# linnanwang/FastGen

Measured on AMD Instinct MI355X. Metric: images/sec at 4-step distilled (DMD2) sampling, higher is better.
Workload: dtype fp32 (tensors, accumulate) with split-bf16 x3 MFMA conv products

## Files before the change

fastgen_amd/csrc/conv.h:

```cpp
#pragma once
#include <hip/hip_runtime.h>

struct ConvArgs {
    const void* src1;
    const void* src2;
    int C1, C2;
    int Hs, Ws;
    int H, W;
    int B;
    const float2* ab;
    const void* wpack;
    const void* wpack_ws;
    const float* bias;
    const float* temb;
    int temb_stride;
    const void* resid;
    float scale;
    void* out;
    int Cout;
    float2* stats;
    int dbg;
    void* q_out;
    void* k_out;
    void* vt_out;
    const float* gate = nullptr;
    int gate_stride = 0;
    int act = 0;
    int heads = 0, head_dim = 0;
    size_t heads_lo_off = 0;
};

enum { PRO_NONE = 0, PRO_GN = 1, PRO_GN_SILU = 2 };
enum { RES_NONE = 0, RES_DOWN = 1, RES_UP = 2 };
enum { OUT_NHWC = 0, OUT_QKV = 1, OUT_TOK = 2, OUT_HEADS = 3 };

int launch_conv_fused(int dtype, int ks, int pro, int res, int outmode, const ConvArgs& a, hipStream_t stream);
int conv_stat_slots(int W);
bool conv_ws_supported(int dtype, int ks, int pro, int res, int outmode, const ConvArgs& a);
bool conv_ws_enabled();
int launch_conv_ws(int res, const ConvArgs& a, hipStream_t stream, bool prepare_only, int pro = PRO_GN_SILU);
bool conv_ws_shape_ok(int dtype, int cout, int cin, int res);
int launch_pack_conv_weights_ws(const float* w_oihw, void* wpack_ws, int cout, int cin, hipStream_t stream);
bool conv_x3ws_supported(int ks, int pro, int res, int outmode, const ConvArgs& a);
bool conv_x3ws_shape_ok(int cout, int cin, int res);
int conv_x3ws_stat_slots(int W);
int launch_conv_x3ws(int res, const ConvArgs& a, hipStream_t stream, bool prepare_only, int pro = PRO_GN_SILU);
int launch_pack_conv_weights_x3ws(const float* w_oihw, void* wpack_ws, int cout, int cin, hipStream_t stream);
int conv_launch_stat_slots(int dtype, int ks, int pro, int res, int outmode, const ConvArgs& a);
int launch_conv_ws_debug(const ConvArgs& a, int abl, hipStream_t stream);
int launch_conv_debug(int dtype, const ConvArgs& a, hipStream_t stream);
int conv_prepare_all(int dtype);
size_t conv_pack_elems(int cout, int cin, int ks);
int launch_pack_conv_weights(int dtype, const float* w_oihw, void* wpack, int cout, int cin, int ks, int qkv_perm,
                             hipStream_t stream);
```

fastgen_amd/csrc/conv_ws3.hip:

```cpp
#include "common.h"
#include "conv.h"

namespace {

constexpr int X3_NTHR = 768;
constexpr int X3_KC = 32;
constexpr int X3_PA = 16;
constexpr int X3_PLANE = 3072;
constexpr int X3_ABUF = 8 * X3_PLANE;
constexpr int X3_RING = 4;
constexpr int X3_HOFF = 128 * 512;
constexpr int X3_LDS = X3_HOFF + X3_RING * X3_ABUF;
constexpr int X3_STEPB = 9 * 2048;

template <int LOGW>
struct X3Geom {
    static constexpr int W = 1 << LOGW;
    static constexpr int TW = 16, TH = 8;
    static constexpr int TCOLS = W / TW;
    static constexpr int TPI = (W / TH) * TCOLS;
    static constexpr int HW_ = TW + 2, HH_ = TH + 2;
    static constexpr int HALO_PIX = HW_ * HH_;
    static constexpr int RS = HW_ * X3_PA;
};

__device__ __forceinline__ void x3_barrier() {
    asm volatile("s_waitcnt lgkmcnt(0)\n\ts_barrier" ::: "memory");
}

struct X3Frag {
    bf16x8 hi, lo;
};

template <int RES, int LOGW, int PRO>
__global__ __launch_bounds__(X3_NTHR) void conv3_x3ws_kernel(const ConvArgs a, const int ntiles) {
    using G = X3Geom<LOGW>;
    extern __shared__ __attribute__((aligned(16))) char smem[];
    char* const hbuf = smem;
    char* const ring = smem + X3_HOFF;

    const int tid = threadIdx.x;
    const int lane = tid & 63;
    const int wave = __builtin_amdgcn_readfirstlane(tid >> 6);
    const int Cin = a.C1 + a.C2;
    const int nchunk = Cin / X3_KC;
    const int G8 = (int)gridDim.x >> 3;
    const int wg = ((gridDim.x & 7) == 0) ? ((int)blockIdx.x & 7) * G8 + ((int)blockIdx.x >> 3) : (int)blockIdx.x;
    const int gstride = (int)gridDim.x;
    const int my_tiles = (ntiles - wg + gstride - 1) / gstride;
    const int S = my_tiles * nchunk;
    const int NSTEP = S + 3;
    const int H = a.H;

    if (wave < 8) {
        const int grp = wave >> 2, wl = wave & 3;
        const int col = lane & 15, g4 = lane >> 4;
        const size_t wstride = (size_t)nchunk * 9 * 1024;
        const __amdgpu_buffer_rsrc_t wrs = __builtin_amdgcn_make_buffer_rsrc(
            const_cast<__bf16*>(reinterpret_cast<const __bf16*>(a.wpack_ws) + (size_t)(grp * 8 + wl * 2) * wstride), 0, 0x7fffffff,
            0x00020000);
        const int wvoff = lane * 16;
        const int wsb = (int)(wstride * 2);
        auto load_w = [&](int byte_off) -> X3Frag {
            X3Frag f;
            f.hi = __builtin_bit_cast(bf16x8, __builtin_amdgcn_raw_buffer_load_b128(wrs, wvoff, byte_off, 0));
            f.lo = __builtin_bit_cast(bf16x8, __builtin_amdgcn_raw_buffer_load_b128(wrs, wvoff, byte_off + 1024, 0));
            return f;
        };
        X3Frag wq[3][2];
#pragma unroll
        for (int j = 0; j < 3; ++j)
#pragma unroll
            for (int nt = 0; nt < 2; ++nt) wq[j][nt] = load_w(nt * wsb + j * 2048);

        f32x4 acc[8][2];
#pragma unroll
        for (int m = 0; m < 8; ++m)
#pragma unroll
            for (int nt = 0; nt < 2; ++nt) acc[m][nt] = f32x4{0.f, 0.f, 0.f, 0.f};

        const int lane_off = g4 * X3_PLANE + col * X3_PA;
        const int dl0 = col * 512 + ((8 * wl + ((g4) ^ (col & 7))) << 4);
        const int dl1 = col * 512 + ((8 * wl + ((4 + g4) ^ (col & 7))) << 4);

        x3_barrier();
        int c = 0;
        for (int s = 0; s < NSTEP; ++s) {
            const int ls = s - 2 * grp;
            if (ls >= 0 && ls < S) {
                const char* abase = ring + (ls & 3) * X3_ABUF + lane_off;
                const int cn = (c + 1 == nchunk) ? 0 : c + 1;
                const int wcur = c * X3_STEPB;
                const int wnxt = (ls + 1 < S) ? cn * X3_STEPB : wcur;
                auto read_x = [&](int q, X3Frag (&xf)[2]) {
                    const int tap = q >> 2, m0 = 2 * (q & 3);
                    const int off = (tap / 3 + m0) * G::RS + (tap % 3) * X3_PA;
#pragma unroll
                    for (int m = 0; m < 2; ++m) {
                        xf[m].hi = *reinterpret_cast<const bf16x8*>(abase + off + m * G::RS);
                        xf[m].lo = *reinterpret_cast<const bf16x8*>(abase + off + m * G::RS + 4 * X3_PLANE);
                    }
                };
                auto mma12 = [&](int q, const X3Frag (&xf)[2]) {
                    const int tap = q >> 2, m0 = 2 * (q & 3);
                    const X3Frag(&wf)[2] = wq[tap % 3];
#pragma unroll
                    for (int m = 0; m < 2; ++m)
#pragma unroll
                        for (int nt = 0; nt < 2; ++nt)
                            acc[m0 + m][nt] = __builtin_amdgcn_mfma_f32_16x16x32_bf16(wf[nt].hi, xf[m].lo, acc[m0 + m][nt], 0, 0, 0);
#pragma unroll
                    for (int m = 0; m < 2; ++m)
#pragma unroll
                        for (int nt = 0; nt < 2; ++nt)
                            acc[m0 + m][nt] = __builtin_amdgcn_mfma_f32_16x16x32_bf16(wf[nt].lo, xf[m].hi, acc[m0 + m][nt], 0, 0, 0);
#pragma unroll
                    for (int m = 0; m < 2; ++m)
#pragma unroll
                        for (int nt = 0; nt < 2; ++nt)
                            acc[m0 + m][nt] = __builtin_amdgcn_mfma_f32_16x16x32_bf16(wf[nt].hi, xf[m].hi, acc[m0 + m][nt], 0, 0, 0);
                    if ((q & 3) != 3) return;
                    const int pn = (tap + 3 < 9) ? wcur + (tap + 3) * 2048 : wnxt + (tap + 3 - 9) * 2048;
#pragma unroll
                    for (int nt = 0; nt < 2; ++nt) wq[tap % 3][nt] = load_w(pn + nt * wsb);
                };
                X3Frag x0[2], x1[2];
                read_x(0, x0);
#pragma unroll
                for (int q = 0; q < 36; q += 2) {
                    read_x(q + 1, x1);
                    __builtin_amdgcn_sched_barrier(0);
                    mma12(q, x0);
                    __builtin_amdgcn_sched_barrier(0);
                    if (q + 2 < 36) read_x(q + 2, x0);
                    __builtin_amdgcn_sched_barrier(0);
                    mma12(q + 1, x1);
                    __builtin_amdgcn_sched_barrier(0);
                }
                if (c + 1 == nchunk) {
#pragma unroll
                    for (int m = 0; m < 8; ++m) {
                        *reinterpret_cast<f32x4*>(hbuf + m * 8192 + dl0) = acc[m][0];
                        *reinterpret_cast<f32x4*>(hbuf + m * 8192 + dl1) = acc[m][1];
                        acc[m][0] = f32x4{0.f, 0.f, 0.f, 0.f};
                        acc[m][1] = f32x4{0.f, 0.f, 0.f, 0.f};
                    }
                }
                c = cn;
            }
            x3_barrier();
        }
        return;
    }

    const int ptid = tid - 512;
    const int pw = wave - 8;
    const int oct = ptid & 3;
    const float* src1 = reinterpret_cast<const float*>(a.src1);
    const float* src2 = reinterpret_cast<const float*>(a.src2);
    int hdy[3], hdx[3], hlds[3];
#pragma unroll
    for (int i = 0; i < 3; ++i) {
        const int hq = min((ptid >> 2) + 64 * i, G::HALO_PIX - 1);
        const int hy = hq / G::HW_, hx = hq - hy * G::HW_;
        hdy[i] = hy - 1;
        hdx[i] = hx - 1;
        hlds[i] = oct * X3_PLANE + hy * G::RS + hx * X3_PA;
    }
    const bool third = (ptid >> 2) + 128 < G::HALO_PIX;

    auto tile_coord = [&](int t, int& n, int& slot, int& row0, int& col0) {
        n = t / G::TPI;
        slot = t - n * G::TPI;
        row0 = (slot / G::TCOLS) * G::TH;
        col0 = (slot % G::TCOLS) * G::TW;
    };

    struct Staged {
        f32x4 raw[3][2];
        float2 ab[8];
    };
    unsigned off1[3], off2[3];
    bool valid[3];
    const float2* abn = a.ab;
    auto tile_setup = [&](int t) __attribute__((always_inline)) {
        int n, slot, row0, col0;
        tile_coord(t, n, slot, row0, col0);
#pragma unroll
        for (int i = 0; i < 3; ++i) {
            const int y = row0 + hdy[i], x = col0 + hdx[i];
            valid[i] = (y >= 0) && (y < H) && (x >= 0) && (x < G::W) && (i < 2 || third);
            const int yc = min(max(y, 0), H - 1), xc = min(max(x, 0), G::W - 1);
            const int sy = (RES == RES_UP) ? (yc >> 1) : yc, sx = (RES == RES_UP) ? (xc >> 1) : xc;
            const unsigned pix = (unsigned)((n * a.Hs + sy) * a.Ws + sx);
            off1[i] = (pix * (unsigned)a.C1 + oct * 8) * 4u;
            off2[i] = (pix * (unsigned)a.C2 + oct * 8) * 4u;
        }
        abn = a.ab + (size_t)n * Cin;
    };
    auto stage_load = [&](Staged& st, int t, int c32) __attribute__((always_inline)) {
        if (c32 == 0) tile_setup(t);
        const bool first = c32 * X3_KC < a.C1;
        const char* base = first ? reinterpret_cast<const char*>(src1) + c32 * (X3_KC * 4)
                                 : reinterpret_cast<const char*>(src2) + (c32 * X3_KC - a.C1) * 4;
#pragma unroll
        for (int i = 0; i < 3; ++i) {
            const char* p = base + (first ? off1[i] : off2[i]);
            st.raw[i][0] = *reinterpret_cast<const f32x4*>(p);
            st.raw[i][1] = *reinterpret_cast<const f32x4*>(p + 16);
        }
        if (PRO == PRO_NONE) return;
        const float2* p = abn + c32 * X3_KC + oct * 8;
#pragma unroll
        for (int j = 0; j < 8; j += 2) {
            const f32x4 q = *reinterpret_cast<const f32x4*>(p + j);
            st.ab[j] = make_float2(q[0], q[1]);
            st.ab[j + 1] = make_float2(q[2], q[3]);
        }
    };
    auto stage_store = [&](const Staged& st, char* abuf) __attribute__((always_inline)) {
#pragma unroll
        for (int i = 0; i < 3; ++i) {
            float v[8];
#pragma unroll
            for (int j = 0; j < 8; ++j) {
                v[j] = st.raw[i][j >> 2][j & 3];
                if (PRO != PRO_NONE) v[j] = silu_f<true>(fmaf(v[j], st.ab[j].x, st.ab[j].y));
            }
            bf16x8 hi, lo;
            split8(v, hi, lo);
            typedef __attribute__((ext_vector_type(4))) unsigned u32x4;
            u32x4 wh = __builtin_bit_cast(u32x4, hi), wl_ = __builtin_bit_cast(u32x4, lo);
#pragma unroll
            for (int j = 0; j < 4; ++j) {
                wh[j] = valid[i] ? wh[j] : 0u;
                wl_[j] = valid[i] ? wl_[j] : 0u;
            }
            if (i < 2 || third) {
                *reinterpret_cast<u32x4*>(abuf + hlds[i]) = wh;
                *reinterpret_cast<u32x4*>(abuf + hlds[i] + 4 * X3_PLANE) = wl_;
            }
        }
    };

    const int chq = lane & 31, psub = lane >> 5;
    float* const out = reinterpret_cast<float*>(a.out);
    const float* const resid = reinterpret_cast<const float*>(a.resid);
    const bool has_resid = __builtin_amdgcn_readfirstlane(resid != nullptr);
    auto retire_half = [&](int t, int half) __attribute__((always_inline)) {
        int n, slot, row0, col0;
        tile_coord(t, n, slot, row0, col0);
        const int co = half * 128 + chq * 4;
        f32x4 radd = {0.f, 0.f, 0.f, 0.f};
        if (a.bias) radd = *reinterpret_cast<const f32x4*>(a.bias + co);
        if (a.temb) radd += *reinterpret_cast<const f32x4*>(a.temb + (size_t)n * a.temb_stride + co);
        radd *= a.scale;
        const size_t tb = (((size_t)n * H + row0) * G::W + col0) * 256 + co;
        float ssum = 0.f, ssq = 0.f;
#pragma unroll 1
        for (int grp8 = 0; grp8 < 2; ++grp8) {
            f32x4 rr[8], dv[8];
            unsigned go[8];
#pragma unroll
            for (int j = 0; j < 8; ++j) {
                const int px = pw * 32 + 2 * (grp8 * 8 + j) + psub;
                go[j] = (unsigned)(((px >> 4) * G::W + (px & 15)) * 256);
                rr[j] = f32x4{0.f, 0.f, 0.f, 0.f};
                if (has_resid) rr[j] = *reinterpret_cast<const f32x4*>(resid + tb + go[j]);
                dv[j] = *reinterpret_cast<const f32x4*>(hbuf + px * 512 + ((chq ^ (px & 7)) << 4));
            }
#pragma unroll
            for (int j = 0; j < 8; ++j) {
                f32x4 v;
#pragma unroll
                for (int e = 0; e < 4; ++e) v[e] = fmaf(dv[j][e], a.scale, radd[e]);
                if (has_resid) {
#pragma unroll
                    for (int e = 0; e < 4; ++e) v[e] = fmaf(rr[j][e], a.scale, v[e]);
                }
                *reinterpret_cast<f32x4*>(out + tb + go[j]) = v;
                ssum += (v[0] + v[1]) + (v[2] + v[3]);
                ssq += (v[0] * v[0] + v[1] * v[1]) + (v[2] * v[2] + v[3] * v[3]);
            }
        }
        ssum += __shfl_xor(ssum, 32);
        ssq += __shfl_xor(ssq, 32);
        if (a.stats && psub == 0) a.stats[(((size_t)n * G::TPI + slot) * 4 + pw) * 64 + half * 32 + chq] = make_float2(ssum, ssq);
    };

    auto advance = [&](int& t, int& cc) {
        if (++cc == nchunk) {
            cc = 0;
            t += gstride;
        }
    };
    Staged st;
    int t1 = wg, c1 = 0;
    stage_load(st, t1, c1);
    stage_store(st, ring);
    advance(t1, c1);
    x3_barrier();
    int sa = 0;
    for (int s = 0; s < NSTEP; ++s) {
        const bool more = s + 1 < S;
        if (more) stage_load(st, t1, c1);
        if (sa == 0 && s >= nchunk && s <= S) retire_half(wg + (s / nchunk - 1) * gstride, 0);
        if (sa == 2 % nchunk && s - 2 >= nchunk && s - 2 <= S && (s - 2) % nchunk == 0) retire_half(wg + ((s - 2) / nchunk - 1) * gstride, 1);
        if (more) {
            stage_store(st, ring + ((s + 1) & 3) * X3_ABUF);
            advance(t1, c1);
        }
        if (++sa == nchunk) sa = 0;
        x3_barrier();
    }
}

__global__ void pack_conv_weights_x3ws_kernel(const float* __restrict__ w, __bf16* __restrict__ out, int cout, int cin) {
    const size_t total = (size_t)cout * cin * 9;
    const int nstep = cin / X3_KC;
    for (size_t idx = (size_t)blockIdx.x * blockDim.x + threadIdx.x; idx < total; idx += (size_t)gridDim.x * blockDim.x) {
        size_t t = idx;
        const int j = t % 8; t /= 8;
        const int lane = t % 64; t /= 64;
        const int tap = t % 9; t /= 9;
        const int step = t % nstep; t /= nstep;
        const int n16 = (int)t;
        const int co = n16 * 16 + (lane & 15);
        const int ci = step * X3_KC + 8 * (lane >> 4) + j;
        const float v = w[((size_t)co * cin + ci) * 9 + tap];
        const __bf16 hi = (__bf16)v;
        const size_t o = (idx / 512) * 1024 + (idx % 512);
        out[o] = hi;
        out[o + 512] = (__bf16)(v - (float)hi);
    }
}

int g_x3_cus[16] = {};

template <int RES, int LOGW, int PRO>
int launch_x3_one(const ConvArgs& a, hipStream_t stream, bool prepare_only) {
    using G = X3Geom<LOGW>;
    auto kern = conv3_x3ws_kernel<RES, LOGW, PRO>;
    int dev = 0;
    if (hipGetDevice(&dev) != hipSuccess || dev < 0 || dev >= 16) return (int)hipErrorInvalidDevice;
    static bool attr_done[16] = {};
    if (!attr_done[dev]) {
        hipError_t e = hipFuncSetAttribute(reinterpret_cast<const void*>(kern), hipFuncAttributeMaxDynamicSharedMemorySize, X3_LDS);
        if (e != hipSuccess) return (int)e;
        attr_done[dev] = true;
    }
    if (!g_x3_cus[dev]) {
        int n = 0;
        if (hipDeviceGetAttribute(&n, hipDeviceAttributeMultiprocessorCount, dev) != hipSuccess || n <= 0) return (int)hipErrorUnknown;
        g_x3_cus[dev] = n;
    }
    if (prepare_only) return 0;
    const int ntiles = a.B * G::TPI;
    const int grid = ntiles < g_x3_cus[dev] ? ntiles : g_x3_cus[dev];
    hipLaunchKernelGGL(kern, dim3(grid), dim3(X3_NTHR), X3_LDS, stream, a, ntiles);
    return (int)hipGetLastError();
}

}

int conv_x3ws_stat_slots(int W) { return (W == 32 ? X3Geom<5>::TPI : X3Geom<4>::TPI) * 4; }

bool conv_x3ws_shape_ok(int cout, int cin, int res) { return cout == 256 && (res == 32 || res == 16) && (cin % X3_KC) == 0 && cin / X3_KC >= 4; }

bool conv_x3ws_supported(int ks, int pro, int res, int outmode, const ConvArgs& a) {
    const int cin = a.C1 + a.C2;
    const size_t src_bytes = (size_t)a.B * a.Hs * a.Ws * (size_t)(a.C1 > a.C2 ? a.C1 : a.C2) * 4;
    if (src_bytes >= (1ull << 32)) return false;
    if (ks != 3 || outmode != OUT_NHWC || a.H != a.W || !conv_x3ws_shape_ok(a.Cout, cin, a.W) || (a.C1 % X3_KC) || !a.wpack_ws) return false;
    if (pro == PRO_NONE) return res == RES_NONE && a.Hs == a.H && a.Ws == a.W;
    return pro == PRO_GN_SILU && (res == RES_NONE || res == RES_UP) && a.ab != nullptr;
}

int launch_conv_x3ws(int res, const ConvArgs& a, hipStream_t stream, bool prepare_only, int pro) {
    if (pro == PRO_NONE) {
        if (res != RES_NONE) return (int)hipErrorInvalidValue;
        return a.W == 32 ? launch_x3_one<RES_NONE, 5, PRO_NONE>(a, stream, prepare_only) : launch_x3_one<RES_NONE, 4, PRO_NONE>(a, stream, prepare_only);
    }
    if (a.W == 32)
        return res == RES_UP ? launch_x3_one<RES_UP, 5, PRO_GN_SILU>(a, stream, prepare_only) : launch_x3_one<RES_NONE, 5, PRO_GN_SILU>(a, stream, prepare_only);
    return res == RES_UP ? launch_x3_one<RES_UP, 4, PRO_GN_SILU>(a, stream, prepare_only) : launch_x3_one<RES_NONE, 4, PRO_GN_SILU>(a, stream, prepare_only);
}

int launch_pack_conv_weights_x3ws(const float* w_oihw, void* wpack_ws, int cout, int cin, hipStream_t stream) {
    const size_t total = (size_t)cout * cin * 9;
    const int grid = (int)((total + 255) / 256 < 4096 ? (total + 255) / 256 : 4096);
    hipLaunchKernelGGL(pack_conv_weights_x3ws_kernel, dim3(grid), dim3(256), 0, stream, w_oihw, (__bf16*)wpack_ws, cout, cin);
    return (int)hipGetLastError();
}
```

fastgen_amd/csrc/engine.hip:

```cpp
#include <hip/hip_runtime.h>

#include <cmath>
#include <cstdarg>
#include <cstdio>
#include <cstdlib>
#include <cstring>
#include <string>
#include <map>
#include <vector>

#include "../../include/fastgen_amd.h"
#include "common.h"
#include "conv.h"
#include "misc.h"

namespace {

thread_local std::string g_err;

int fail(int code, const char* fmt, ...) {
    char buf[512];
    va_list ap;
    va_start(ap, fmt);
    vsnprintf(buf, sizeof buf, fmt, ap);
    va_end(ap);
    g_err = buf;
    return code;
}

#define HIP_TRY(expr)                                                                                          \
    do {                                                                                                       \
        hipError_t e_ = (hipError_t)(expr);                                                                    \
        if (e_ != hipSuccess) return fail(FG_EHIP, "%s failed: %s (%s:%d)", #expr, hipGetErrorString(e_), __FILE__, __LINE__); \
    } while (0)

struct Param {
    std::string name;
    int ndim = 0;
    int64_t shape[4] = {1, 1, 1, 1};
    int64_t numel = 0;
    const float* ptr = nullptr;
    float* grad = nullptr;
};

enum Kind { K_STEM, K_BLOCK, K_AUX_NORM, K_AUX_CONV };

struct Block {
    std::string key;
    Kind kind = K_BLOCK;
    int cin = 0, cout = 0, res_in = 0, res_out = 0;
    bool up = false, down = false, attn = false, has_skip = false, is_dec = false;
    int skip_c = 0;
    int temb_off = 0;
    int norm0_w = -1, norm0_b = -1, conv0_w = -1, conv0_b = -1, aff_w = -1, aff_b = -1, norm1_w = -1, norm1_b = -1,
        conv1_w = -1, conv1_b = -1, skip_w = -1, skip_b = -1, norm2_w = -1, norm2_b = -1, qkv_w = -1, qkv_b = -1,
        proj_w = -1, proj_b = -1, w = -1, b = -1;
    void *p_conv0 = nullptr, *p_conv1 = nullptr, *p_skip = nullptr, *p_qkv = nullptr, *p_proj = nullptr;
    void *p_conv0_ws = nullptr, *p_conv1_ws = nullptr;
    int tap = -1;
    float* qkv_bias = nullptr;
    void* p_aux = nullptr;
    void* p_stem = nullptr;
};

struct Arena {
    char* base = nullptr;
    size_t off = 0, cap = 0;
    bool dry = false;
    void* take(size_t bytes) {
        off = (off + 255) & ~(size_t)255;
        void* p = dry ? nullptr : base + off;
        off += bytes;
        return p;
    }
    template <typename T>
    T* get(size_t n) {
        return reinterpret_cast<T*>(take(n * sizeof(T)));
    }
};

struct Act {
    void* p = nullptr;
    float2* st = nullptr;
    int slots = 0;
};

struct Workspace {
    float *coef, *emb0, *emb1, *emb, *temb;
    float2 *ab0, *ab1, *ab2;
    float2 *mr0 = nullptr, *mr1 = nullptr, *mr2 = nullptr;
    void* a1d = nullptr;
    DropArgs drop;
    std::vector<Act> skip;
    Act xa, xb, h, xattn;
    void *sbuf, *aout, *pool;
    void *cvt1, *cvt2;
    void *q, *k, *vt;
    float *x, *x_pred, *eps;
    double* tl;
    uint64_t* seed;
};

struct BlockStash {
    void* h = nullptr;
    float2 *ab0 = nullptr, *ab1 = nullptr, *ab2 = nullptr, *mr0 = nullptr, *mr1 = nullptr, *mr2 = nullptr;
    void *xattn = nullptr, *q = nullptr, *k = nullptr, *vt = nullptr, *aout = nullptr;
    void* a1d = nullptr;
    uint32_t index = 0;
};
struct TrainStash {
    std::vector<Act> dec_store;
// ... 302 lines not shown
        if (hipEventCreate(&e0) != hipSuccess || hipEventCreate(&e1) != hipSuccess) return (int)hipErrorUnknown;
        (void)hipEventRecord(e0, s);
    }
    const int rc = launch_conv_fused(h->cmode, ks, pro, res, outmode, a, s);
    if (timed) {
        (void)hipEventRecord(e1, s);
        h->prof_ev.push_back(e0);
        h->prof_ev.push_back(e1);
        h->prof_flops += 2.0 * a.B * a.H * a.W * (double)a.Cout * 9.0 * (a.C1 + a.C2);
    }
    return rc;
}

const float kSkipScale = (float)std::sqrt(0.5);
const float kBlockEps = 1e-6f;

int norm_coeffs(int dtype, const Act& x1, int c1, const Act& x2, int c2, const float* gamma, const float* beta, float2* ab,
                int B, int hw, hipStream_t s, float2* mr = nullptr) {
    if (x1.st && (!c2 || x2.st))
        HIP_TRY(launch_gn_finalize(x1.st, c1, x1.slots, c2 ? x2.st : nullptr, c2, c2 ? x2.slots : 0, gamma, beta, kBlockEps, ab, B, hw, s, mr));
    else
        HIP_TRY(launch_gn_coeffs(dtype, x1.p, c1, c2 ? x2.p : nullptr, c2, gamma, beta, kBlockEps, ab, B, hw, s, mr));
    return FG_OK;
}

void use_stash(Workspace& w, const BlockStash& st) {
    w.h.p = st.h;
    w.ab0 = st.ab0, w.ab1 = st.ab1, w.mr0 = st.mr0, w.mr1 = st.mr1;
    w.a1d = st.a1d;
    w.drop.block = st.index;
    if (st.xattn) {
        w.xattn.p = st.xattn;
        w.ab2 = st.ab2, w.mr2 = st.mr2;
        w.q = st.q, w.k = st.k, w.vt = st.vt, w.aout = st.aout;
    }
}
int block_index(const fg_edm* h, const Block* b) {
    for (size_t i = 0; i < h->blocks.size(); ++i)
        if (h->blocks[i] == b) return (int)i;
    return -1;
}

int run_block(fg_edm* h, const Block& b, const Act& x1, int c1, const Act& x2, int c2, const float* temb, Act& out, int B,
              Workspace& w, hipStream_t s) {
    if (c1 + c2 != b.cin) return fail(FG_EINVAL, "%s: got %d+%d input channels, expected %d", b.key.c_str(), c1, c2, b.cin);
    const int hw_in = b.res_in * b.res_in, hw = b.res_out * b.res_out;
    const int res_mode = b.down ? RES_DOWN : (b.up ? RES_UP : RES_NONE);
    const int slots = conv_stat_slots(b.res_out);
    int rc;
    if ((rc = norm_coeffs(h->dtype, x1, c1, x2, c2, h->P(b.norm0_w), h->P(b.norm0_b), w.ab0, B, hw_in, s, w.mr0))) return rc;
    ConvArgs a{};
    a.src1 = x1.p; a.src2 = c2 ? x2.p : nullptr; a.C1 = c1; a.C2 = c2;
    a.Hs = a.Ws = b.res_in; a.H = a.W = b.res_out; a.B = B;
    a.ab = w.ab0; a.wpack = b.p_conv0; a.wpack_ws = b.p_conv0_ws; a.bias = h->P(b.conv0_b);
    a.temb = temb + b.temb_off; a.temb_stride = h->temb_total;
    a.resid = nullptr; a.scale = 1.0f; a.out = w.h.p; a.Cout = b.cout; a.stats = w.h.st;
    if (b.down && !c2) {
        HIP_TRY(launch_gn_silu_pool(h->dtype, x1.p, w.ab0, w.pool, B, b.res_out, b.res_out, c1, s));
        a.src1 = w.pool; a.Hs = a.Ws = b.res_out; a.ab = nullptr;
        w.h.slots = conv_launch_stat_slots(h->cmode, 3, PRO_NONE, RES_NONE, OUT_NHWC, a);
        HIP_TRY(conv_launch(h, 3, PRO_NONE, RES_NONE, OUT_NHWC, a, s));
    } else {
        w.h.slots = conv_launch_stat_slots(h->cmode, 3, PRO_GN_SILU, res_mode, OUT_NHWC, a);
        HIP_TRY(conv_launch(h, 3, PRO_GN_SILU, res_mode, OUT_NHWC, a, s));
    }
    const void* resid = x1.p;
    if (b.has_skip) {
        ConvArgs k{};
        k.src1 = x1.p; k.src2 = c2 ? x2.p : nullptr; k.C1 = c1; k.C2 = c2;
        k.Hs = k.Ws = b.res_in; k.H = k.W = b.res_out; k.B = B;
        k.wpack = b.p_skip; k.bias = h->P(b.skip_b); k.scale = 1.0f; k.out = w.sbuf; k.Cout = b.cout;
        HIP_TRY(conv_launch(h, 1, PRO_NONE, res_mode, OUT_NHWC, k, s));
        resid = w.sbuf;
    }
    HIP_TRY(launch_gn_finalize(w.h.st, b.cout, w.h.slots, nullptr, 0, 0, h->P(b.norm1_w), h->P(b.norm1_b), kBlockEps, w.ab1, B, hw, s, w.mr1));
    Act& x_mid = b.attn ? w.xattn : out;
    ConvArgs d{};
    d.src1 = w.h.p; d.C1 = b.cout; d.Hs = d.Ws = d.H = d.W = b.res_out; d.B = B;
    d.ab = w.ab1; d.wpack = b.p_conv1; d.wpack_ws = b.p_conv1_ws; d.bias = h->P(b.conv1_b);
    d.resid = resid; d.scale = kSkipScale; d.out = x_mid.p; d.Cout = b.cout; d.stats = x_mid.st;
    if (w.a1d) {
        HIP_TRY(launch_gn_act(h->dtype, 0, w.h.p, b.cout, nullptr, 0, w.ab1, w.a1d, B, b.res_out, 0, s, w.drop));
        d.src1 = w.a1d; d.ab = nullptr;
        x_mid.slots = conv_launch_stat_slots(h->cmode, 3, PRO_NONE, RES_NONE, OUT_NHWC, d);
        HIP_TRY(conv_launch(h, 3, PRO_NONE, RES_NONE, OUT_NHWC, d, s));
    } else {
        x_mid.slots = conv_launch_stat_slots(h->cmode, 3, PRO_GN_SILU, RES_NONE, OUT_NHWC, d);
        HIP_TRY(conv_launch(h, 3, PRO_GN_SILU, RES_NONE, OUT_NHWC, d, s));
    }
    if (b.attn) {
        HIP_TRY(launch_gn_finalize(x_mid.st, b.cout, x_mid.slots, nullptr, 0, 0, h->P(b.norm2_w), h->P(b.norm2_b), kBlockEps, w.ab2, B, hw, s, w.mr2));
        ConvArgs q{};
        q.src1 = x_mid.p; q.C1 = b.cout; q.Hs = q.Ws = q.H = q.W = b.res_out; q.B = B;
        q.ab = w.ab2; q.wpack = b.p_qkv; q.bias = b.qkv_bias; q.scale = 1.0f; q.Cout = 3 * b.cout;
        q.q_out = w.q; q.k_out = w.k; q.vt_out = w.vt;
        HIP_TRY(conv_launch(h, 1, PRO_GN, RES_NONE, OUT_QKV, q, s));
        HIP_TRY(launch_attention(h->cmode, w.q, w.k, w.vt, w.aout, B, hw, s));
        ConvArgs p{};
        p.src1 = w.aout; p.C1 = b.cout; p.Hs = p.Ws = p.H = p.W = b.res_out; p.B = B;
        p.wpack = b.p_proj; p.bias = h->P(b.proj_b); p.resid = x_mid.p; p.scale = kSkipScale; p.out = out.p; p.Cout = b.cout;
        p.stats = out.st;
        HIP_TRY(conv_launch(h, 1, PRO_NONE, RES_NONE, OUT_NHWC, p, s));
        out.slots = slots;
    }
    return FG_OK;
}

// ... 98 lines not shown
                if ((rc = sde_noise(i, &e))) return rc;
                HIP_TRY(launch_forward_process(w.x, e, 0.0, w.tl, i + 1, sched, w.x, total, s));
            }
        }
        return FG_OK;
    }
    for (int i = 0; i < steps; ++i) {
        float* pred = (i == steps - 1) ? out : w.x_pred;
        int rc = run_forward(h, w.x, w.tl + i, 0, w.tl + steps, 0, labels, pred, B, w, s);
        if (rc) return rc;
        if (t_list[i + 1] > 0) {
            const float* e = nullptr;
            if (type == FG_SAMPLE_SDE) {
                if ((rc = sde_noise(i, &e))) return rc;
            } else {
                HIP_TRY(launch_x0_to_eps(w.x, pred, 0.0, w.tl, i, sched, 1e-6, w.eps, total, s));
                e = w.eps;
            }
            HIP_TRY(launch_forward_process(pred, e, 0.0, w.tl, i + 1, sched, w.x, total, s));
        }
    }
    return FG_OK;
}

void drop_graph(fg_edm* h) {
    if (h->graph_exec) (void)hipGraphExecDestroy(h->graph_exec);
    if (h->graph) (void)hipGraphDestroy(h->graph);
    h->graph_exec = nullptr;
    h->graph = nullptr;
}

int setup_ws(const fg_edm* h, int B, void* workspace, size_t bytes, Workspace& w) {
    if (B <= 0) return fail(FG_EINVAL, "batch must be positive");
    if (!workspace) return fail(FG_EINVAL, "workspace is null");
    if (((uintptr_t)workspace) & 255) return fail(FG_EINVAL, "workspace must be 256-byte aligned");
    Arena A;
    A.base = (char*)workspace;
    const size_t need = plan_workspace(h, B, A, w);
    if (need > bytes) return fail(FG_ENOMEM, "workspace too small: need %zu bytes for batch %d, got %zu", need, B, bytes);
    return FG_OK;
}

int ensure_device_state(fg_edm* h) {
    if (h->device_ready) return FG_OK;
    int rc;
    const size_t tsz = h->dtype ? 2 : 4;
    for (Block* b : h->blocks) {
        if ((rc = dev_alloc(h, &b->p_conv0, conv_pack_elems(b->cout, b->cin, 3) * tsz))) return rc;
        if ((rc = dev_alloc(h, &b->p_conv1, conv_pack_elems(b->cout, b->cout, 3) * tsz))) return rc;
        const bool x3 = h->cmode == FG_DTYPE_BF16X3;
        if ((x3 ? conv_x3ws_shape_ok(b->cout, b->cin, b->res_out) : conv_ws_shape_ok(h->cmode, b->cout, b->cin, b->res_out)) && !b->down &&
            (rc = dev_alloc(h, &b->p_conv0_ws, conv_pack_elems(b->cout, b->cin, 3) * tsz)))
            return rc;
        if ((x3 ? conv_x3ws_shape_ok(b->cout, b->cout, b->res_out) : conv_ws_shape_ok(h->cmode, b->cout, b->cout, b->res_out)) &&
            (rc = dev_alloc(h, &b->p_conv1_ws, conv_pack_elems(b->cout, b->cout, 3) * tsz)))
            return rc;
        if (b->has_skip && (rc = dev_alloc(h, &b->p_skip, conv_pack_elems(b->cout, b->cin, 1) * tsz))) return rc;
        if (b->attn) {
            if ((rc = dev_alloc(h, &b->p_qkv, conv_pack_elems(3 * b->cout, b->cout, 1) * tsz))) return rc;
            if ((rc = dev_alloc(h, &b->p_proj, conv_pack_elems(b->cout, b->cout, 1) * tsz))) return rc;
            if ((rc = dev_alloc(h, (void**)&b->qkv_bias, sizeof(float) * 3 * b->cout))) return rc;
        }
    }
    for (Block& b : h->enc)
        if (b.kind == K_STEM && stem_supported(b.res_out, b.cin, b.cout))
            if ((rc = dev_alloc(h, &b.p_stem, stem_pack_elems() * tsz))) return rc;
    for (Block& b : h->dec)
        if (b.kind == K_AUX_CONV && aux_head_supported(h->cmode, b.res_out, b.cin, b.cout))
            if ((rc = dev_alloc(h, &b.p_aux, aux_pack_elems(b.cin) * tsz))) return rc;
    if ((rc = dev_alloc(h, (void**)&h->aff_w, sizeof(float) * (size_t)h->temb_total * h->emb_ch))) return rc;
    if ((rc = dev_alloc(h, (void**)&h->aff_b, sizeof(float) * (size_t)h->temb_total))) return rc;
    const int half = h->noise_ch / 2;
    std::vector<float> fr(half);
    for (int j = 0; j < half; ++j) fr[j] = powf(1.0f / 10000.0f, (float)j / (float)(half - 1));
    if ((rc = dev_alloc(h, (void**)&h->freqs, sizeof(float) * half))) return rc;
    HIP_TRY(hipMemcpy(h->freqs, fr.data(), sizeof(float) * half, hipMemcpyHostToDevice));
    if (conv_prepare_all(h->cmode) != 0) return fail(FG_EHIP, "hipFuncSetAttribute(dynamic LDS) failed");
    if (launch_attention(h->cmode, nullptr, nullptr, nullptr, nullptr, 1, 256, nullptr) != 0) return fail(FG_EHIP, "attention prepare failed");
    HIP_TRY(hipHostMalloc((void**)&h->slots, sizeof(fg_edm::Slot) * fg_edm::kSlots));
    for (int i = 0; i < fg_edm::kSlots; ++i) HIP_TRY(hipEventCreateWithFlags(&h->slot_ev[i], hipEventDisableTiming));
    h->device_ready = true;
    return FG_OK;
}

}

extern "C" {

const char* fg_last_error(void) { return g_err.c_str(); }
const char* fg_version(void) { return "fastgen_amd 0.1 gfx950"; }

int fg_edm_create(const fg_edm_config* cfg, fg_edm** out) {
    if (!cfg || !out) return fail(FG_EINVAL, "null argument");
    if (cfg->num_levels < 1 || cfg->num_levels > FG_MAX_LEVELS || cfg->num_attn_resolutions < 0 ||
        cfg->num_attn_resolutions > FG_MAX_LEVELS)
        return fail(FG_EINVAL, "bad num_levels / num_attn_resolutions");
    if (cfg->compute_dtype != FG_DTYPE_F32 && cfg->compute_dtype != FG_DTYPE_BF16 && cfg->compute_dtype != FG_DTYPE_BF16X3)
        return fail(FG_EINVAL, "bad compute_dtype");
    if ((cfg->drop_precond & ~3) || (cfg->schedule != FG_SCHEDULE_EDM && cfg->schedule != FG_SCHEDULE_RF) ||
        (cfg->r_timestep & ~1))
        return fail(FG_EINVAL, "bad r_timestep / drop_precond / schedule");
    if (cfg->model_channels <= 0 || cfg->model_channels % 16 || cfg->channel_mult_noise < 1 || cfg->channel_mult_emb < 1)
        return fail(FG_EINVAL, "bad channel configuration");
    fg_edm* h = new fg_edm();
    h->cfg = *cfg;
    h->cmode = cfg->compute_dtype;
// ... 11 lines not shown
    return FG_OK;
}

void fg_edm_destroy(fg_edm* h) {
    if (!h) return;
    drop_graph(h);
    for (void* p : h->owned) (void)hipFree(p);
    if (h->slots) (void)hipHostFree(h->slots);
    for (hipEvent_t e : h->slot_ev)
        if (e) (void)hipEventDestroy(e);
    if (h->cap_stream) (void)hipStreamDestroy(h->cap_stream);
    for (hipEvent_t e : h->prof_ev) (void)hipEventDestroy(e);
    delete h;
}

int fg_edm_num_params(const fg_edm* h) { return h ? (int)h->params.size() : 0; }

int fg_edm_param_info(const fg_edm* h, int index, const char** name, int* ndim, int64_t shape[4]) {
    if (!h || index < 0 || index >= (int)h->params.size()) return fail(FG_EINVAL, "param index out of range");
    const Param& p = h->params[index];
    if (name) *name = p.name.c_str();
    if (ndim) *ndim = p.ndim;
    if (shape)
        for (int i = 0; i < 4; ++i) shape[i] = p.shape[i];
    return FG_OK;
}

int fg_edm_bind_param(fg_edm* h, const char* name, const float* device_ptr, int64_t numel) {
    if (!h || !name || !device_ptr) return fail(FG_EINVAL, "null argument");
    const int i = h->find(name);
    if (i < 0) return fail(FG_EINVAL, "unknown parameter '%s'", name);
    if (h->params[i].numel != numel)
        return fail(FG_EINVAL, "parameter '%s': expected %lld elements, got %lld", name, (long long)h->params[i].numel, (long long)numel);
    h->params[i].ptr = device_ptr;
    h->packed = false;
    return FG_OK;
}

int fg_edm_pack_weights(fg_edm* h, void* stream) {
    if (!h) return fail(FG_EINVAL, "null handle");
    hipStream_t s = (hipStream_t)stream;
    int rc0 = ensure_device_state(h);
    if (rc0) return rc0;
    for (const Param& p : h->params) {
        const bool unused = (p.name == "model.map_augment.weight" && !h->augment) || p.name.rfind("model.logvar_linear", 0) == 0;
        if (!p.ptr && !unused) return fail(FG_ENOTREADY, "parameter '%s' is not bound", p.name.c_str());
    }
    ++h->pack_epoch;
    for (Block* b : h->blocks) {
        HIP_TRY(launch_pack_conv_weights(h->cmode, h->P(b->conv0_w), b->p_conv0, b->cout, b->cin, 3, 0, s));
        HIP_TRY(launch_pack_conv_weights(h->cmode, h->P(b->conv1_w), b->p_conv1, b->cout, b->cout, 3, 0, s));
        if (h->cmode == FG_DTYPE_BF16X3) {
            if (b->p_conv0_ws) HIP_TRY(launch_pack_conv_weights_x3ws(h->P(b->conv0_w), b->p_conv0_ws, b->cout, b->cin, s));
            if (b->p_conv1_ws) HIP_TRY(launch_pack_conv_weights_x3ws(h->P(b->conv1_w), b->p_conv1_ws, b->cout, b->cout, s));
        } else {
            if (b->p_conv0_ws) HIP_TRY(launch_pack_conv_weights_ws(h->P(b->conv0_w), b->p_conv0_ws, b->cout, b->cin, s));
            if (b->p_conv1_ws) HIP_TRY(launch_pack_conv_weights_ws(h->P(b->conv1_w), b->p_conv1_ws, b->cout, b->cout, s));
        }
        if (b->has_skip) HIP_TRY(launch_pack_conv_weights(h->cmode, h->P(b->skip_w), b->p_skip, b->cout, b->cin, 1, 0, s));
        if (b->attn) {
            HIP_TRY(launch_pack_conv_weights(h->cmode, h->P(b->qkv_w), b->p_qkv, 3 * b->cout, b->cout, 1, 1, s));
            HIP_TRY(launch_pack_conv_weights(h->cmode, h->P(b->proj_w), b->p_proj, b->cout, b->cout, 1, 0, s));
            for (int plane = 0; plane < 3; ++plane)
                HIP_TRY(hipMemcpy2DAsync(b->qkv_bias + plane * b->cout, sizeof(float), h->P(b->qkv_b) + plane,
                                         3 * sizeof(float), sizeof(float), b->cout, hipMemcpyDeviceToDevice, s));
        }
        HIP_TRY(hipMemcpyAsync(h->aff_w + (size_t)b->temb_off * h->emb_ch, h->P(b->aff_w),
                               sizeof(float) * (size_t)b->cout * h->emb_ch, hipMemcpyDeviceToDevice, s));
        HIP_TRY(hipMemcpyAsync(h->aff_b + b->temb_off, h->P(b->aff_b), sizeof(float) * b->cout, hipMemcpyDeviceToDevice, s));
    }
    for (Block& b : h->enc)
        if (b.kind == K_STEM && b.p_stem) HIP_TRY(launch_pack_stem_weights(h->dtype, h->P(b.w), b.p_stem, b.cin, s));
    for (Block& b : h->dec)
        if (b.kind == K_AUX_CONV && b.p_aux) HIP_TRY(launch_pack_aux_weights(h->cmode, h->P(b.w), b.p_aux, b.cin, b.cout, s));
    drop_graph(h);
    h->packed = true;
    return FG_OK;
}

size_t fg_edm_workspace_bytes(const fg_edm* h, int batch) {
    if (!h || batch <= 0) return 0;
    Arena A;
    A.dry = true;
    Workspace w;
    return plan_workspace(h, batch, A, w);
}

int fg_edm_forward(fg_edm* h, const float* x_t, const double* t, const double* r, const float* class_labels, float* out,
                   float* emb_out, int batch, void* workspace, size_t workspace_bytes, void* stream) {
    if (!h || !x_t || !t || !out) return fail(FG_EINVAL, "null argument");
    if (r && !h->cfg.r_timestep) return fail(FG_EINVAL, "r_noise_labels provided, but r_timestep is not set");
    if (!r && h->cfg.r_timestep) return fail(FG_EINVAL, "this network was built with r_timestep: r is required");
    if (!h->packed) return fail(FG_ENOTREADY, "weights are not packed (call fg_edm_pack_weights)");
    if (out == x_t) return fail(FG_EINVAL, "out must not alias x_t");
    Workspace w;
    int rc = setup_ws(h, batch, workspace, workspace_bytes, w);
    if (rc) return rc;
    hipStream_t s = (hipStream_t)stream;
    rc = run_forward(h, x_t, t, 1, r, 1, class_labels, out, batch, w, s);
    if (rc) return rc;
    if (emb_out) HIP_TRY(hipMemcpyAsync(emb_out, w.emb, sizeof(float) * (size_t)batch * h->emb_ch, hipMemcpyDeviceToDevice, s));
    return FG_OK;
}

int fg_edm_num_feature_taps(const fg_edm* h) { return h ? h->num_taps : 0; }

// ... 423 lines not shown
```

Measured before the change: 2711.

## Fold nearest-upsample into 3x3 conv via phase-decomposed 2x2 summed weights

For the upsampling conv0 path, the 3x3 conv over a 2x nearest-upsampled input is rewritten as four phase-specific 2x2 convs on the low-res input, with weights pre-summed at pack time into 16 taps. This cuts MFMA work from 9 to 4 taps per output pixel and shrinks the input halo that is staged into LDS. The tile geometry, LDS addressing, output pixel mapping and weight ring are templated for the UP case, and an extra packed weight buffer is allocated. Summing the weights before bf16 splitting changes rounding slightly.

```diff
diff --git a/fastgen_amd/csrc/conv.h b/fastgen_amd/csrc/conv.h
--- a/fastgen_amd/csrc/conv.h
+++ b/fastgen_amd/csrc/conv.h
@@ -11,6 +11,7 @@
     const float2* ab;
     const void* wpack;
     const void* wpack_ws;
+    const void* wpack_up;
     const float* bias;
     const float* temb;
     int temb_stride;
@@ -45,7 +46,8 @@
 bool conv_x3ws_shape_ok(int cout, int cin, int res);
 int conv_x3ws_stat_slots(int W);
 int launch_conv_x3ws(int res, const ConvArgs& a, hipStream_t stream, bool prepare_only, int pro = PRO_GN_SILU);
-int launch_pack_conv_weights_x3ws(const float* w_oihw, void* wpack_ws, int cout, int cin, hipStream_t stream);
+int launch_pack_conv_weights_x3ws(const float* w_oihw, void* wpack_ws, int cout, int cin, hipStream_t stream, bool up = false);
+size_t conv_x3ws_up_pack_bytes(int cout, int cin);
 int conv_launch_stat_slots(int dtype, int ks, int pro, int res, int outmode, const ConvArgs& a);
 int launch_conv_ws_debug(const ConvArgs& a, int abl, hipStream_t stream);
 int launch_conv_debug(int dtype, const ConvArgs& a, hipStream_t stream);
diff --git a/fastgen_amd/csrc/conv_ws3.hip b/fastgen_amd/csrc/conv_ws3.hip
--- a/fastgen_amd/csrc/conv_ws3.hip
+++ b/fastgen_amd/csrc/conv_ws3.hip
@@ -11,17 +11,24 @@
 constexpr int X3_RING = 4;
 constexpr int X3_HOFF = 128 * 512;
 constexpr int X3_LDS = X3_HOFF + X3_RING * X3_ABUF;
-constexpr int X3_STEPB = 9 * 2048;
-
-template <int LOGW>
+
+template <int LOGW, bool UP = false>
 struct X3Geom {
     static constexpr int W = 1 << LOGW;
     static constexpr int TW = 16, TH = 8;
     static constexpr int TCOLS = W / TW;
     static constexpr int TPI = (W / TH) * TCOLS;
-    static constexpr int HW_ = TW + 2, HH_ = TH + 2;
+    static constexpr int HW_ = (UP ? TW / 2 : TW) + 2, HH_ = (UP ? TH / 2 : TH) + 2;
     static constexpr int HALO_PIX = HW_ * HH_;
-    static constexpr int RS = HW_ * X3_PA;
+    static constexpr int NIT = (HALO_PIX + 63) / 64;
+    static constexpr int RS = UP ? 384 : HW_ * X3_PA;
+    static constexpr int NTAP = UP ? 16 : 9;
+    static constexpr int QPT = UP ? 1 : 4;
+    static constexpr int NQ = NTAP * QPT;
+    static constexpr int STEPB = NTAP * 2048;
+    static constexpr int WR = UP ? 4 : 3;
+    static_assert(NTAP % WR == 0, "the weight ring must wrap at step boundaries");
+    static_assert(HH_ * RS <= X3_PLANE, "halo plane overflows");
 };
 
 __device__ __forceinline__ void x3_barrier() {
@@ -34,7 +41,8 @@
 
 template <int RES, int LOGW, int PRO>
 __global__ __launch_bounds__(X3_NTHR) void conv3_x3ws_kernel(const ConvArgs a, const int ntiles) {
-    using G = X3Geom<LOGW>;
+    constexpr bool UP = RES == RES_UP;
+    using G = X3Geom<LOGW, UP>;
     extern __shared__ __attribute__((aligned(16))) char smem[];
     char* const hbuf = smem;
     char* const ring = smem + X3_HOFF;
@@ -55,9 +63,9 @@
     if (wave < 8) {
         const int grp = wave >> 2, wl = wave & 3;
         const int col = lane & 15, g4 = lane >> 4;
-        const size_t wstride = (size_t)nchunk * 9 * 1024;
+        const size_t wstride = (size_t)nchunk * G::NTAP * 1024;
         const __amdgpu_buffer_rsrc_t wrs = __builtin_amdgcn_make_buffer_rsrc(
-            const_cast<__bf16*>(reinterpret_cast<const __bf16*>(a.wpack_ws) + (size_t)(grp * 8 + wl * 2) * wstride), 0, 0x7fffffff,
+            const_cast<__bf16*>(reinterpret_cast<const __bf16*>(UP ? a.wpack_up : a.wpack_ws) + (size_t)(grp * 8 + wl * 2) * wstride), 0, 0x7fffffff,
             0x00020000);
         const int wvoff = lane * 16;
         const int wsb = (int)(wstride * 2);
@@ -67,9 +75,9 @@
             f.lo = __builtin_bit_cast(bf16x8, __builtin_amdgcn_raw_buffer_load_b128(wrs, wvoff, byte_off + 1024, 0));
             return f;
         };
-        X3Frag wq[3][2];
-#pragma unroll
-        for (int j = 0; j < 3; ++j)
+        X3Frag wq[G::WR][2];
+#pragma unroll
+        for (int j = 0; j < G::WR; ++j)
 #pragma unroll
             for (int nt = 0; nt < 2; ++nt) wq[j][nt] = load_w(nt * wsb + j * 2048);
 
@@ -79,7 +87,7 @@
 #pragma unroll
             for (int nt = 0; nt < 2; ++nt) acc[m][nt] = f32x4{0.f, 0.f, 0.f, 0.f};
 
-        const int lane_off = g4 * X3_PLANE + col * X3_PA;
+        const int lane_off = g4 * X3_PLANE + (UP ? (col >> 3) * G::RS + (col & 7) * X3_PA : col * X3_PA);
         const int dl0 = col * 512 + ((8 * wl + ((g4) ^ (col & 7))) << 4);
         const int dl1 = col * 512 + ((8 * wl + ((4 + g4) ^ (col & 7))) << 4);
 
@@ -90,20 +98,25 @@
             if (ls >= 0 && ls < S) {
                 const char* abase = ring + (ls & 3) * X3_ABUF + lane_off;
                 const int cn = (c + 1 == nchunk) ? 0 : c + 1;
-                const int wcur = c * X3_STEPB;
-                const int wnxt = (ls + 1 < S) ? cn * X3_STEPB : wcur;
+                const int wcur = c * G::STEPB;
+                const int wnxt = (ls + 1 < S) ? cn * G::STEPB : wcur;
+                auto x_off = [&](int q) {
+                    if (UP) return (((q >> 1) & 1) + (q >> 3)) * G::RS + ((q & 1) + ((q >> 2) & 1)) * X3_PA;
+                    const int tap = q >> 2;
+                    return (tap / 3 + 2 * (q & 3)) * G::RS + (tap % 3) * X3_PA;
+                };
+                constexpr int MS = UP ? 2 * G::RS : G::RS;
                 auto read_x = [&](int q, X3Frag (&xf)[2]) {
-                    const int tap = q >> 2, m0 = 2 * (q & 3);
-                    const int off = (tap / 3 + m0) * G::RS + (tap % 3) * X3_PA;
+                    const int off = x_off(q);
 #pragma unroll
                     for (int m = 0; m < 2; ++m) {
-                        xf[m].hi = *reinterpret_cast<const bf16x8*>(abase + off + m * G::RS);
-                        xf[m].lo = *reinterpret_cast<const bf16x8*>(abase + off + m * G::RS + 4 * X3_PLANE);
+                        xf[m].hi = *reinterpret_cast<const bf16x8*>(abase + off + m * MS);
+                        xf[m].lo = *reinterpret_cast<const bf16x8*>(abase + off + m * MS + 4 * X3_PLANE);
                     }
                 };
                 auto mma12 = [&](int q, const X3Frag (&xf)[2]) {
-                    const int tap = q >> 2, m0 = 2 * (q & 3);
-                    const X3Frag(&wf)[2] = wq[tap % 3];
+                    const int tap = q / G::QPT, m0 = UP ? 2 * (q >> 2) : 2 * (q & 3);
+                    const X3Frag(&wf)[2] = wq[tap % G::WR];
 #pragma unroll
                     for (int m = 0; m < 2; ++m)
 #pragma unroll
@@ -119,20 +132,20 @@
 #pragma unroll
                         for (int nt = 0; nt < 2; ++nt)
                             acc[m0 + m][nt] = __builtin_amdgcn_mfma_f32_16x16x32_bf16(wf[nt].hi, xf[m].hi, acc[m0 + m][nt], 0, 0, 0);
-                    if ((q & 3) != 3) return;
-                    const int pn = (tap + 3 < 9) ? wcur + (tap + 3) * 2048 : wnxt + (tap + 3 - 9) * 2048;
-#pragma unroll
-                    for (int nt = 0; nt < 2; ++nt) wq[tap % 3][nt] = load_w(pn + nt * wsb);
+                    if (q % G::QPT != G::QPT - 1) return;
+                    const int pn = (tap + G::WR < G::NTAP) ? wcur + (tap + G::WR) * 2048 : wnxt + (tap + G::WR - G::NTAP) * 2048;
+#pragma unroll
+                    for (int nt = 0; nt < 2; ++nt) wq[tap % G::WR][nt] = load_w(pn + nt * wsb);
                 };
                 X3Frag x0[2], x1[2];
                 read_x(0, x0);
 #pragma unroll
-                for (int q = 0; q < 36; q += 2) {
+                for (int q = 0; q < G::NQ; q += 2) {
                     read_x(q + 1, x1);
                     __builtin_amdgcn_sched_barrier(0);
                     mma12(q, x0);
                     __builtin_amdgcn_sched_barrier(0);
-                    if (q + 2 < 36) read_x(q + 2, x0);
+                    if (q + 2 < G::NQ) read_x(q + 2, x0);
                     __builtin_amdgcn_sched_barrier(0);
                     mma12(q + 1, x1);
                     __builtin_amdgcn_sched_barrier(0);
@@ -158,16 +171,17 @@
     const int oct = ptid & 3;
     const float* src1 = reinterpret_cast<const float*>(a.src1);
     const float* src2 = reinterpret_cast<const float*>(a.src2);
-    int hdy[3], hdx[3], hlds[3];
-#pragma unroll
-    for (int i = 0; i < 3; ++i) {
+    constexpr int NIT = G::NIT;
+    int hdy[NIT], hdx[NIT], hlds[NIT];
+#pragma unroll
+    for (int i = 0; i < NIT; ++i) {
         const int hq = min((ptid >> 2) + 64 * i, G::HALO_PIX - 1);
         const int hy = hq / G::HW_, hx = hq - hy * G::HW_;
         hdy[i] = hy - 1;
         hdx[i] = hx - 1;
         hlds[i] = oct * X3_PLANE + hy * G::RS + hx * X3_PA;
     }
-    const bool third = (ptid >> 2) + 128 < G::HALO_PIX;
+    const bool last = (ptid >> 2) + 64 * (NIT - 1) < G::HALO_PIX;
 
     auto tile_coord = [&](int t, int& n, int& slot, int& row0, int& col0) {
         n = t / G::TPI;
@@ -177,21 +191,22 @@
     };
 
     struct Staged {
-        f32x4 raw[3][2];
+        f32x4 raw[NIT][2];
         float2 ab[8];
     };
-    unsigned off1[3], off2[3];
-    bool valid[3];
+    unsigned off1[NIT], off2[NIT];
+    bool valid[NIT];
     const float2* abn = a.ab;
     auto tile_setup = [&](int t) __attribute__((always_inline)) {
         int n, slot, row0, col0;
         tile_coord(t, n, slot, row0, col0);
-#pragma unroll
-        for (int i = 0; i < 3; ++i) {
+        const int sh = UP ? a.Hs : H, sw = UP ? a.Ws : G::W;
+        if (UP) row0 >>= 1, col0 >>= 1;
+#pragma unroll
+        for (int i = 0; i < NIT; ++i) {
             const int y = row0 + hdy[i], x = col0 + hdx[i];
-            valid[i] = (y >= 0) && (y < H) && (x >= 0) && (x < G::W) && (i < 2 || third);
-            const int yc = min(max(y, 0), H - 1), xc = min(max(x, 0), G::W - 1);
-            const int sy = (RES == RES_UP) ? (yc >> 1) : yc, sx = (RES == RES_UP) ? (xc >> 1) : xc;
+            valid[i] = (y >= 0) && (y < sh) && (x >= 0) && (x < sw) && (i < NIT - 1 || last);
+            const int sy = min(max(y, 0), sh - 1), sx = min(max(x, 0), sw - 1);
             const unsigned pix = (unsigned)((n * a.Hs + sy) * a.Ws + sx);
             off1[i] = (pix * (unsigned)a.C1 + oct * 8) * 4u;
             off2[i] = (pix * (unsigned)a.C2 + oct * 8) * 4u;
@@ -204,7 +219,7 @@
         const char* base = first ? reinterpret_cast<const char*>(src1) + c32 * (X3_KC * 4)
                                  : reinterpret_cast<const char*>(src2) + (c32 * X3_KC - a.C1) * 4;
 #pragma unroll
-        for (int i = 0; i < 3; ++i) {
+        for (int i = 0; i < NIT; ++i) {
             const char* p = base + (first ? off1[i] : off2[i]);
             st.raw[i][0] = *reinterpret_cast<const f32x4*>(p);
             st.raw[i][1] = *reinterpret_cast<const f32x4*>(p + 16);
@@ -220,7 +235,7 @@
     };
     auto stage_store = [&](const Staged& st, char* abuf) __attribute__((always_inline)) {
 #pragma unroll
-        for (int i = 0; i < 3; ++i) {
+        for (int i = 0; i < NIT; ++i) {
             float v[8];
 #pragma unroll
             for (int j = 0; j < 8; ++j) {
@@ -236,7 +251,7 @@
                 wh[j] = valid[i] ? wh[j] : 0u;
                 wl_[j] = valid[i] ? wl_[j] : 0u;
             }
-            if (i < 2 || third) {
+            if (i < NIT - 1 || last) {
                 *reinterpret_cast<u32x4*>(abuf + hlds[i]) = wh;
                 *reinterpret_cast<u32x4*>(abuf + hlds[i] + 4 * X3_PLANE) = wl_;
             }
@@ -264,7 +279,9 @@
 #pragma unroll
             for (int j = 0; j < 8; ++j) {
                 const int px = pw * 32 + 2 * (grp8 * 8 + j) + psub;
-                go[j] = (unsigned)(((px >> 4) * G::W + (px & 15)) * 256);
+                const int oy = UP ? 4 * ((px >> 4) & 1) + 2 * ((px >> 3) & 1) + (px >> 6) : px >> 4;
+                const int ox = UP ? 2 * (px & 7) + ((px >> 5) & 1) : px & 15;
+                go[j] = (unsigned)((oy * G::W + ox) * 256);
                 rr[j] = f32x4{0.f, 0.f, 0.f, 0.f};
                 if (has_resid) rr[j] = *reinterpret_cast<const f32x4*>(resid + tb + go[j]);
                 dv[j] = *reinterpret_cast<const f32x4*>(hbuf + px * 512 + ((chq ^ (px & 7)) << 4));
@@ -315,19 +332,32 @@
     }
 }
 
+template <bool UP>
 __global__ void pack_conv_weights_x3ws_kernel(const float* __restrict__ w, __bf16* __restrict__ out, int cout, int cin) {
-    const size_t total = (size_t)cout * cin * 9;
+    constexpr int NTAP = UP ? 16 : 9;
+    const size_t total = (size_t)cout * cin * NTAP;
     const int nstep = cin / X3_KC;
     for (size_t idx = (size_t)blockIdx.x * blockDim.x + threadIdx.x; idx < total; idx += (size_t)gridDim.x * blockDim.x) {
         size_t t = idx;
         const int j = t % 8; t /= 8;
         const int lane = t % 64; t /= 64;
-        const int tap = t % 9; t /= 9;
+        const int tap = t % NTAP; t /= NTAP;
         const int step = t % nstep; t /= nstep;
         const int n16 = (int)t;
         const int co = n16 * 16 + (lane & 15);
         const int ci = step * X3_KC + 8 * (lane >> 4) + j;
-        const float v = w[((size_t)co * cin + ci) * 9 + tap];
+        const float* wk = w + ((size_t)co * cin + ci) * 9;
+        float v;
+        if (UP) {
+            const int dy = tap >> 3, dx = (tap >> 2) & 1, ty = (tap >> 1) & 1, tx = tap & 1;
+            const int ky0 = (dy == 0) ? (ty ? 1 : 0) : (ty ? 2 : 0), ky1 = (dy == 0) ? (ty ? 2 : 0) : (ty ? 2 : 1);
+            const int kx0 = (dx == 0) ? (tx ? 1 : 0) : (tx ? 2 : 0), kx1 = (dx == 0) ? (tx ? 2 : 0) : (tx ? 2 : 1);
+            v = 0.f;
+            for (int ky = ky0; ky <= ky1; ++ky)
+                for (int kx = kx0; kx <= kx1; ++kx) v += wk[ky * 3 + kx];
+        } else {
+            v = wk[tap];
+        }
         const __bf16 hi = (__bf16)v;
         const size_t o = (idx / 512) * 1024 + (idx % 512);
         out[o] = hi;
@@ -373,6 +403,7 @@
     if (src_bytes >= (1ull << 32)) return false;
     if (ks != 3 || outmode != OUT_NHWC || a.H != a.W || !conv_x3ws_shape_ok(a.Cout, cin, a.W) || (a.C1 % X3_KC) || !a.wpack_ws) return false;
     if (pro == PRO_NONE) return res == RES_NONE && a.Hs == a.H && a.Ws == a.W;
+    if (res == RES_UP && (!a.wpack_up || 2 * a.Hs != a.H || 2 * a.Ws != a.W)) return false;
     return pro == PRO_GN_SILU && (res == RES_NONE || res == RES_UP) && a.ab != nullptr;
 }
 
@@ -386,9 +417,12 @@
     return res == RES_UP ? launch_x3_one<RES_UP, 4, PRO_GN_SILU>(a, stream, prepare_only) : launch_x3_one<RES_NONE, 4, PRO_GN_SILU>(a, stream, prepare_only);
 }
 
-int launch_pack_conv_weights_x3ws(const float* w_oihw, void* wpack_ws, int cout, int cin, hipStream_t stream) {
-    const size_t total = (size_t)cout * cin * 9;
+int launch_pack_conv_weights_x3ws(const float* w_oihw, void* wpack_ws, int cout, int cin, hipStream_t stream, bool up) {
+    const size_t total = (size_t)cout * cin * (up ? 16 : 9);
     const int grid = (int)((total + 255) / 256 < 4096 ? (total + 255) / 256 : 4096);
-    hipLaunchKernelGGL(pack_conv_weights_x3ws_kernel, dim3(grid), dim3(256), 0, stream, w_oihw, (__bf16*)wpack_ws, cout, cin);
+    hipLaunchKernelGGL(up ? pack_conv_weights_x3ws_kernel<true> : pack_conv_weights_x3ws_kernel<false>, dim3(grid), dim3(256), 0, stream,
+                       w_oihw, (__bf16*)wpack_ws, cout, cin);
     return (int)hipGetLastError();
 }
+
+size_t conv_x3ws_up_pack_bytes(int cout, int cin) { return (size_t)cout * cin * 16 * 4; }
diff --git a/fastgen_amd/csrc/engine.hip b/fastgen_amd/csrc/engine.hip
--- a/fastgen_amd/csrc/engine.hip
+++ b/fastgen_amd/csrc/engine.hip
@@ -57,6 +57,7 @@
         proj_w = -1, proj_b = -1, w = -1, b = -1;
     void *p_conv0 = nullptr, *p_conv1 = nullptr, *p_skip = nullptr, *p_qkv = nullptr, *p_proj = nullptr;
     void *p_conv0_ws = nullptr, *p_conv1_ws = nullptr;
+    void* p_conv0_up = nullptr;
     int tap = -1;
     float* qkv_bias = nullptr;
     void* p_aux = nullptr;
@@ -465,7 +466,7 @@
     ConvArgs a{};
     a.src1 = x1.p; a.src2 = c2 ? x2.p : nullptr; a.C1 = c1; a.C2 = c2;
     a.Hs = a.Ws = b.res_in; a.H = a.W = b.res_out; a.B = B;
-    a.ab = w.ab0; a.wpack = b.p_conv0; a.wpack_ws = b.p_conv0_ws; a.bias = h->P(b.conv0_b);
+    a.ab = w.ab0; a.wpack = b.p_conv0; a.wpack_ws = b.p_conv0_ws; a.wpack_up = b.p_conv0_up; a.bias = h->P(b.conv0_b);
     a.temb = temb + b.temb_off; a.temb_stride = h->temb_total;
     a.resid = nullptr; a.scale = 1.0f; a.out = w.h.p; a.Cout = b.cout; a.stats = w.h.st;
     if (b.down && !c2) {
@@ -670,6 +671,7 @@
         if ((x3 ? conv_x3ws_shape_ok(b->cout, b->cin, b->res_out) : conv_ws_shape_ok(h->cmode, b->cout, b->cin, b->res_out)) && !b->down &&
             (rc = dev_alloc(h, &b->p_conv0_ws, conv_pack_elems(b->cout, b->cin, 3) * tsz)))
             return rc;
+        if (x3 && b->up && b->p_conv0_ws && (rc = dev_alloc(h, &b->p_conv0_up, conv_x3ws_up_pack_bytes(b->cout, b->cin)))) return rc;
         if ((x3 ? conv_x3ws_shape_ok(b->cout, b->cout, b->res_out) : conv_ws_shape_ok(h->cmode, b->cout, b->cout, b->res_out)) &&
             (rc = dev_alloc(h, &b->p_conv1_ws, conv_pack_elems(b->cout, b->cout, 3) * tsz)))
             return rc;
@@ -787,6 +789,7 @@
         HIP_TRY(launch_pack_conv_weights(h->cmode, h->P(b->conv1_w), b->p_conv1, b->cout, b->cout, 3, 0, s));
         if (h->cmode == FG_DTYPE_BF16X3) {
             if (b->p_conv0_ws) HIP_TRY(launch_pack_conv_weights_x3ws(h->P(b->conv0_w), b->p_conv0_ws, b->cout, b->cin, s));
+            if (b->p_conv0_up) HIP_TRY(launch_pack_conv_weights_x3ws(h->P(b->conv0_w), b->p_conv0_up, b->cout, b->cin, s, true));
             if (b->p_conv1_ws) HIP_TRY(launch_pack_conv_weights_x3ws(h->P(b->conv1_w), b->p_conv1_ws, b->cout, b->cout, s));
         } else {
             if (b->p_conv0_ws) HIP_TRY(launch_pack_conv_weights_ws(h->P(b->conv0_w), b->p_conv0_ws, b->cout, b->cin, s));
```

Measured after the change: 2736 (median of 6 runs). No clear change (+0.9%).
